# ciccio42/openvla-oft

Hardware: AMD Instinct MI355X
Metric: fine-tune samples/s (action-chunks/s) OpenVLA-7B bf16 (higher is better)
Workload: dtype bf16; 1 GPU; BASELINE.json configs[2]: LoRA r=32 fine-tune step (fwd+bwd+AdamW), 2x224x224 images + proprio, L1 head; global_batch=8, seq_len=608, parallelism=dp1, mask_mode=bidirectional

## Files before the change

### include/ovla.h

```cpp
#ifndef OVLA_H_
#define OVLA_H_

#include <stdint.h>

#ifdef __cplusplus
extern "C" {
#endif

#define OVLA_OK 0
#define OVLA_EINVAL (-1)
#define OVLA_EARCH (-2)
#define OVLA_ELAUNCH (-3)

#define OVLA_ABI_VERSION 1

const char* ovla_last_error(void);
int ovla_abi_version(void);
const char* ovla_build_hash(void);
int ovla_check_device(int device);

enum { OVLA_ACT_NONE = 0, OVLA_ACT_GELU = 1, OVLA_ACT_RELU = 2, OVLA_ACT_SILU = 3, OVLA_ACT_GELU_TANH = 4,
       OVLA_ACT_SWIGLU = 5 };

typedef struct {
  const void* A; int64_t lda;
  const void* B; int64_t ldb;
  const void* A2; int64_t lda2;
  const void* B2; int64_t ldb2;
  void* C; int64_t ldc;
  void* C_pre;
  const void* bias;
  const void* colscale;
  const void* residual; int64_t ldr;
  const void* film_gamma;
  const void* film_beta;
  int32_t film_rows;
  int32_t M, N, K, K2;
  int32_t k2_group_n;
  int32_t a_group_n;
  int32_t act;
  int32_t split_k;
  int32_t tile;
  float alpha;
  const void* dact_src; int64_t ld_dact;
  int32_t dact_mode, dact_act;
  const void* rope_cos; const void* rope_sin;
  int32_t rope_S, rope_cols;
  float* rowsq_out;
  const float* rowscale_part; int32_t rowscale_slots; float rowscale_eps; float* rowscale_r;
  uint32_t* hybrid_counters; int32_t n_hybrid_counters;
  void* workspace;
  int64_t workspace_bytes;
} ovla_gemm_args;

int ovla_gemm_plan(int32_t M, int32_t N, int32_t K, int32_t K2, int32_t k2_group_n, int64_t workspace_bytes, int32_t* tile,
                   int32_t* full_tiles, int32_t* rem_tiles, int32_t* rem_splits, double* est_seconds);
int ovla_gemm_resolved_tile(const ovla_gemm_args* a, int32_t* tile);
int64_t ovla_gemm_workspace_bytes(int32_t M, int32_t N, int32_t split_k);
int ovla_gemm_bf16(const ovla_gemm_args* a, void* stream);

typedef struct {
  int32_t tile;
  int32_t splits;
} ovla_gemm_schedule;
enum { OVLA_EPI_ROPE = 1,
       OVLA_EPI_ROWSCALE = 2,
       OVLA_EPI_SWIGLU = 4,
       OVLA_EPI_GENERAL = 8,
       OVLA_EPI_ROWSQ = 16     };
int ovla_gemm_fixed_schedule(int32_t N, int32_t K, int32_t K2, int32_t k2_group_n, int32_t epi_flags, ovla_gemm_schedule* out);
int64_t ovla_gemm_fixed_workspace_bytes(int32_t M, int32_t N, const ovla_gemm_schedule* s);
int ovla_gemm_bf16_fixed(const ovla_gemm_args* a, const ovla_gemm_schedule* s, void* stream);

typedef struct {
  const void* X; int64_t ldx;
  const void* Y; int64_t ldy;
  void* C; int64_t ldc;
  int32_t M, P, Q;
  float alpha;
  int32_t out_mode;
  float* W;
} ovla_gemm_tn_args;
int64_t ovla_gemm_tn_workspace_floats(const ovla_gemm_tn_args* a, int32_t group_size);
int ovla_gemm_tn_bf16(const ovla_gemm_tn_args* a, void* stream);
#define OVLA_TN_MAX_GROUP 4
int ovla_gemm_tn_grouped(const ovla_gemm_tn_args* problems, int32_t n, void* stream);

typedef struct {
  const void* dy; int64_t ld_dy;
  const void* Bt; int64_t ld_bt;
  const void* t;  int64_t ld_t;
  void* dt; int64_t ld_dt;
  float* dB; int64_t ld_db;
  int32_t M, gn, G, r;
  float scale;
  void* workspace; int64_t workspace_bytes;
} ovla_lora_bwd_args;
int64_t ovla_lora_bwd_workspace_bytes(int32_t M, int32_t gn, int32_t G);
int ovla_lora_bwd(const ovla_lora_bwd_args* a, void* stream);

typedef struct {
  void* t; int64_t ld;
  const int32_t* obs_slot;
  const int32_t* obs_slot_host;
  int32_t M, G, n, r, rows_per_obs, n_obs;
} ovla_lora_route_args;
int ovla_lora_route(const ovla_lora_route_args* a, void* stream);

typedef struct {
  const void* src; void* dst;
  const int32_t* obs_slot; const int32_t* obs_slot_host;
  int64_t src_slot_stride;
  int32_t n, rows, dim, rows_per_obs, n_obs, elem_bytes;
} ovla_select_by_slot_args;
int ovla_select_by_slot(const ovla_select_by_slot_args* a, void* stream);

typedef struct { const void* X; int64_t ldx; float* out; int32_t M, N; } ovla_colsum_args;
int ovla_colsum_bf16(const ovla_colsum_args* a, void* stream);

typedef struct {
  const void* Q; const void* K; const void* V; int64_t q_stride, k_stride, v_stride;
  void* O; int64_t o_stride;
  float* lse;
  const int32_t* kv_len;
  int32_t B, H, S, head_dim;
  int32_t causal;
  float scale;
} ovla_attn_fwd_args;
int ovla_attn_fwd(const ovla_attn_fwd_args* a, void* stream);

typedef struct {
  const void* Q; const void* K; const void* V; int64_t q_stride, k_stride, v_stride;
  const void* O; const void* dO; int64_t o_stride, do_stride;
  const float* lse;
  float* delta;
  void* dQ; void* dK; void* dV; int64_t dq_stride, dk_stride, dv_stride;
  const int32_t* kv_len;
  int32_t B, H, S, head_dim;
  int32_t causal;
  float scale;
  const void* rope_cos;
  const void* rope_sin;
} ovla_attn_bwd_args;
int ovla_attn_bwd(const ovla_attn_bwd_args* a, void* stream);

typedef struct {
  const void* x; void* y; const void* weight; const void* bias;
  float* mean; float* rstd;
  int32_t rows, dim; float eps; int32_t is_rms;
} ovla_norm_fwd_args;
int ovla_norm_fwd(const ovla_norm_fwd_args* a, void* stream);

typedef struct {
  const void* x; const void* dy; const void* weight;
  const float* mean; const float* rstd;
  void* dx; float* dweight; float* dbias;
  int32_t rows, dim; int32_t is_rms; int32_t dx_accum;
} ovla_norm_bwd_args;
int ovla_norm_bwd(const ovla_norm_bwd_args* a, void* stream);

int ovla_rope_table(void* cos_table, void* sin_table, int32_t S, int32_t head_dim, float theta, void* stream);
typedef struct {
  void* qk; int64_t ld; int32_t rows, S, n_heads, head_dim;
  const void* cos_table; const void* sin_table; int32_t inverse;
} ovla_rope_args;
int ovla_rope(const ovla_rope_args* a, void* stream);

typedef struct { const void* gu; void* h; int32_t rows, F; } ovla_swiglu_fwd_args;
int ovla_swiglu_fwd(const ovla_swiglu_fwd_args* a, void* stream);
typedef struct { const void* gu; const void* dh; void* dgu; int32_t rows, F; } ovla_swiglu_bwd_args;
int ovla_swiglu_bwd(const ovla_swiglu_bwd_args* a, void* stream);

typedef struct { const void* z; const void* dh; void* dz; int64_t n; int32_t act; } ovla_act_bwd_args;
int ovla_act_bwd(const ovla_act_bwd_args* a, void* stream);

typedef struct { const void* a; const void* b; void* out; int64_t n; } ovla_add_args;
int ovla_add_bf16(const ovla_add_args* a, void* stream);
typedef struct { const void* x; const void* scale; void* out; int32_t rows, dim; } ovla_colscale_args;
int ovla_colscale_bf16(const ovla_colscale_args* a, void* stream);

typedef struct { const void* pixels; void* out; int64_t ldo; int32_t B, C_total, c0, H, W, patch, n_img, img_cstride; } ovla_im2col_args;
int ovla_im2col(const ovla_im2col_args* a, void* stream);

typedef struct { const void* src; void* dst; int32_t n_img, H, W, out, crop; float crop_scale; float mean[6]; float std[6]; } ovla_image_prep_args;
int ovla_image_prep(const ovla_image_prep_args* a, void* stream);

typedef struct {
  const void* src; void* dst; void* workspace; int64_t workspace_bytes;
  const int32_t* row_starts; const float* row_weights; const int32_t* col_starts; const float* col_weights;
  int32_t n_img, H, W, out_h, out_w, row_span, col_span;
} ovla_image_resize_args;
int64_t ovla_image_resize_workspace_bytes(int32_t n_img, int32_t W, int32_t out_h);
int ovla_image_resize(const ovla_image_resize_args* a, void* stream);

typedef struct { const void* src; void* dst; void* workspace; int64_t workspace_bytes; int32_t n_img, H, W, quality; } ovla_jpeg_roundtrip_args;
int64_t ovla_jpeg_roundtrip_workspace_bytes(int32_t n_img, int32_t H, int32_t W);
int ovla_jpeg_roundtrip(const ovla_jpeg_roundtrip_args* a, void* stream);

typedef struct {
  const void* src; void* dst; const float* params; void* workspace; int64_t workspace_bytes;
  int32_t n_img, H, W, out, ops_mask; float mean[6]; float std[6];
} ovla_image_augment_args;
int64_t ovla_image_augment_workspace_bytes(int32_t n_img, int32_t out);
int ovla_image_augment(const ovla_image_augment_args* a, void* stream);

typedef struct { const void* patches; const void* pos; const void* prefix; void* tokens; int32_t B, n_patches, n_prefix, dim; } ovla_vit_embed_args;
int ovla_vit_embed(const ovla_vit_embed_args* a, void* stream);
typedef struct {
  const void* src; void* dst; int32_t B, rows, dim;
  int64_t src_batch_stride, src_row0, src_ld, dst_batch_stride, dst_row0, dst_ld, dst_col0; int32_t accumulate;
} ovla_copy_rows_args;
int ovla_copy_rows(const ovla_copy_rows_args* a, void* stream);

typedef struct { void* dy; const void* x_pre; const void* gamma; float* dgamma; float* dbeta; int32_t B, rows_per_batch, dim; } ovla_film_bwd_args;
int ovla_film_bwd(const ovla_film_bwd_args* a, void* stream);

typedef struct { const void* x; const uint8_t* row_mask; void* out; int32_t B, L, dim; } ovla_masked_mean_args;
int ovla_masked_mean(const ovla_masked_mean_args* a, void* stream);

typedef struct { const int64_t* ids; const int64_t* labels; const void* embed_table; void* out; int32_t B, L, D, vocab; int64_t action_token_begin; } ovla_language_average_args;
int ovla_language_average(const ovla_language_average_args* a, void* stream);

typedef struct { const int64_t* ids; const int64_t* labels; const int32_t* lens; const void* embed_table; void* out; int32_t B, L, D, vocab; int64_t action_token_begin; } ovla_language_average_ragged_args;
int ovla_language_average_ragged(const ovla_language_average_ragged_args* a, void* stream);

typedef struct {
  const int64_t* ids; const int64_t* labels;
  const void* embed_table;
  const void* patches;
  const void* noisy;
  void* out;
  int32_t* action_pos;
  int32_t B, L, P, D, A, vocab;
  int32_t ignore_index, action_token_begin, action_dim;
} ovla_assemble_args;
int ovla_assemble_multimodal(const ovla_assemble_args* a, void* stream);

int ovla_row_sumsq(const void* x, int64_t ld, float* out, int32_t rows, int32_t dim, void* stream);

typedef struct { const void* src; const int32_t* index; void* dst; int32_t n, dim; int64_t src_ld, dst_ld; int32_t scatter_add; } ovla_gather_rows_args;
int ovla_gather_rows(const ovla_gather_rows_args* a, void* stream);

typedef struct {
  const void* logits; int64_t ld; const int64_t* targets; float* loss_rows; int32_t* argmax; void* dlogits; int64_t ld_d;
  int32_t rows, vocab; float grad_scale;
} ovla_token_ce_args;
int ovla_token_ce(const ovla_token_ce_args* a, void* stream);

typedef struct { const void* logits; int64_t ld; int32_t* token; int32_t* bin; int32_t rows, vocab, n_tokens, n_bins; } ovla_argmax_bins_args;
int ovla_argmax_bins(const ovla_argmax_bins_args* a, void* stream);

typedef struct {
  const void* x; const void* W; const void* b; void* pred;
  const void* target; float* loss_sum;
// ... 57 lines not shown
```

### openvla-oft_amd/engine.py

```python
from __future__ import annotations

import contextlib
import math
from typing import Dict, List, Optional

import os

import torch

from . import _lib, ops
from .config import VLAConfig, VitConfig

BF16 = torch.bfloat16
F32 = torch.float32
_FUSE = os.environ.get("OVLA_FUSE_DACT", "none")
_FUSE_ROPE_FWD = os.environ.get("OVLA_FUSE_ROPE_FWD", "1") == "1"
_GROUP_TN = os.environ.get("OVLA_GROUP_TN", "1") == "1"
_FUSE_ACT, _FUSE_SWIGLU = _FUSE in ("act", "all"), _FUSE in ("swiglu", "all")
_FUSE_HEAD = {"0": False, "1": True}.get(os.environ.get("OVLA_FUSE_HEAD", "auto"), None)
_ASYNC_UPLOAD = os.environ.get("OVLA_ASYNC_UPLOAD", "1") != "0"
_FOLD_RMSNORM = os.environ.get("OVLA_FOLD_RMSNORM", "1") != "0"
_INFER_W4 = os.environ.get("OVLA_INFER_W4", "1") != "0"
_FUSE_SWIGLU_FWD = os.environ.get("OVLA_FUSE_SWIGLU_FWD", "0") == "1"
_LORA_BWD_FUSED = os.environ.get("OVLA_LORA_BWD", "0") == "1"


class Param:

    def __init__(self, name, init: torch.Tensor):
        self.name, self.shape, self.dtype = name, tuple(init.shape), init.dtype
        self._init = init
        self.data: Optional[torch.Tensor] = None
        self.grad: Optional[torch.Tensor] = None
        self.offset = 0

    @property
    def numel(self):
        return math.prod(self.shape)


class ParamStore:
    ALIGN = 64

    def __init__(self, device):
        self.device = device
        self.params: List[Param] = []
        self.flat: Dict[torch.dtype, torch.Tensor] = {}
        self.flat_grad: Dict[torch.dtype, torch.Tensor] = {}
        self.exp_avg: Dict[torch.dtype, torch.Tensor] = {}
        self.exp_avg_sq: Dict[torch.dtype, torch.Tensor] = {}
        self.step = 0
        self.finalized = False

    def add(self, name: str, init: torch.Tensor) -> Param:
        assert not self.finalized and init.dtype in (BF16, F32)
        p = Param(name, init.to(self.device))
        self.params.append(p)
        return p

    def finalize(self):
        for dtype in (BF16, F32):
            group = [p for p in reversed(self.params) if p.dtype == dtype]
            total = 0
            for p in group:
                p.offset = total
                total += (p.numel + self.ALIGN - 1) // self.ALIGN * self.ALIGN
            if total == 0:
                continue
            flat = torch.zeros(total, dtype=dtype, device=self.device)
            grad = torch.zeros(total, dtype=F32, device=self.device)
            for p in group:
                p.data = flat[p.offset: p.offset + p.numel].view(p.shape)
                p.data.copy_(p._init)
                p.grad = grad[p.offset: p.offset + p.numel].view(p.shape)
                p._init = None
            self.flat[dtype], self.flat_grad[dtype] = flat, grad
        self.finalized = True

    def init_optimizer(self):
        for dtype, flat in self.flat.items():
            self.exp_avg[dtype] = torch.zeros_like(flat)
            self.exp_avg_sq[dtype] = torch.zeros_like(flat)
        self.step = 0

    def zero_grad(self):
        for g in self.flat_grad.values():
            g.zero_()

    def adamw_step(self, lr: float, *, beta1=0.9, beta2=0.999, eps=1e-8, weight_decay=0.01, grad_scale=1.0):
        if not self.exp_avg:
            self.init_optimizer()
        self.step += 1
        for dtype, flat in self.flat.items():
            ops.adamw(flat, self.exp_avg[dtype], self.exp_avg_sq[dtype], self.flat_grad[dtype], step=self.step, lr=lr, beta1=beta1,
                      beta2=beta2, eps=eps, weight_decay=weight_decay, grad_scale=grad_scale)

    def num_trainable(self):
        return sum(p.numel for p in self.params)

    def named(self) -> Dict[str, Param]:
        return {p.name: p for p in self.params}


MAX_SLOTS = 4


def slot_a_rows(g: int, s: int, n: int, r: int) -> slice:
    return slice((g * n + s) * r, (g * n + s + 1) * r)


def fill_slot(A_slots, B_slots, s: int, lora_A, lora_B, groups: int):
    r = lora_B.shape[1]
    n = B_slots.shape[1] // r
    for g in range(groups):
        A_slots[slot_a_rows(g, s, n, r)] = lora_A[g * r:(g + 1) * r].to(A_slots.device, A_slots.dtype)
    B_slots[:, s * r:(s + 1) * r] = lora_B.to(B_slots.device, B_slots.dtype)


class SlotRoute:

    def __init__(self):
        self.obs_slot: Optional[torch.Tensor] = None
        self.n_obs = 0
        self.host_slots: Optional[List[int]] = None


class SlotProjectors:

    def __init__(self, comps, route: SlotRoute):
        self.comps, self.route = list(comps), route

    def fwd(self, x, train: bool):
        assert not train, "multi-policy serving is inference-only"
        ys = torch.stack([c.fwd(x, False)[0] for c in self.comps])
        out = torch.zeros_like(ys[0])
        B = self.route.n_obs
        ops.select_by_slot(ys, self.route.obs_slot, rows_per_obs=1, rows=B, out=out[:B], host_slots=self.route.host_slots)
        return out, None


class LoraLinear:

    def __init__(self, store: Optional[ParamStore], name: str, W: torch.Tensor, bias: Optional[torch.Tensor], lora_A: Optional[torch.Tensor],
                 lora_B: Optional[torch.Tensor], groups: int, scale: float, need_dgrad: bool = True, ref_names=None):
        self.name, self.W, self.bias, self.groups, self.scale = name, W.contiguous(), bias, groups, scale
        self.ref_names = ref_names or [name]
        self.out_f, self.in_f = W.shape
        self.group_n = self.out_f // groups
        self.WT = ops.transpose(self.W) if need_dgrad else None
        self.has_lora = lora_A is not None
        if self.has_lora:
            self.r = lora_A.shape[0] // groups
            assert lora_A.shape == (groups * self.r, self.in_f) and lora_B.shape == (self.out_f, self.r)
            self.A = store.add(name + ".lora_A", lora_A.to(BF16))
            self.B = store.add(name + ".lora_B", lora_B.to(BF16))
            self.AT = None
            self.BT = None

    def derived_pairs(self):
        if not self.has_lora:
            return []
        dev = self.W.device
        if self.AT is None:
            self.AT = torch.empty((self.in_f, self.groups * self.r), dtype=BF16, device=dev)
            self.BT = torch.empty((self.groups * self.r, self.group_n), dtype=BF16, device=dev)
        pairs = [(self.A.data, self.AT)]
        for g in range(self.groups):
            pairs.append((self.B.data[g * self.group_n:(g + 1) * self.group_n], self.BT[g * self.r:(g + 1) * self.r]))
        return pairs

    def refresh_derived(self):
        for src, dst in self.derived_pairs():
            ops.transpose(src, dst)

    def export(self, kind: str = "data") -> Dict[str, torch.Tensor]:
        out = {}
        if self.has_lora:
            A, Bm = getattr(self.A, kind), getattr(self.B, kind)
            for g, rn in enumerate(self.ref_names):
                out[rn + ".lora_A.weight"] = A[g * self.r:(g + 1) * self.r]
                out[rn + ".lora_B.weight"] = Bm[g * self.group_n:(g + 1) * self.group_n]
        return out

    def merge(self):
        if not self.has_lora or getattr(self, "merged", False):
            return
        if self.AT is None:
            self.refresh_derived()
        gn, r = self.group_n, self.r
        for g in range(self.groups):
            Wg = self.W[g * gn:(g + 1) * gn]
            ops.gemm(self.B.data[g * gn:(g + 1) * gn], self.AT[:, g * r:(g + 1) * r], out=Wg, residual=Wg, alpha=self.scale)
        if self.WT is not None:
            ops.transpose(self.W, self.WT)
        self.merged = True

    def init_slots(self, n: int, r: int, route: "SlotRoute"):
        if self.has_lora:
            raise ValueError(f"{self.name}: adapter slots need a linear without merged or trainable adapters")
        if not 1 <= n <= MAX_SLOTS:
            raise ValueError(f"{self.name}: {n} adapter slots (1 .. {MAX_SLOTS} supported)")
        if r % 8:
            raise ValueError(f"{self.name}: slot rank {r} must be a multiple of 8")
        dev = self.W.device
        self.n_slots, self.slot_r, self.route = n, r, route
        self.A_slots = torch.zeros((self.groups * n * r, self.in_f), dtype=BF16, device=dev)
        self.B_slots = torch.zeros((self.out_f, n * r), dtype=BF16, device=dev)

    def clear_slots(self):
        self.n_slots, self.A_slots, self.B_slots = 0, None, None

    def set_slot(self, s: int, lora_A: torch.Tensor, lora_B: torch.Tensor):
        n, r, G = self.n_slots, self.slot_r, self.groups
        if not 0 <= s < n:
            raise ValueError(f"{self.name}: slot {s} of {n}")
        if tuple(lora_A.shape) != (G * r, self.in_f) or tuple(lora_B.shape) != (self.out_f, r):
            raise ValueError(f"{self.name}: adapter shapes {tuple(lora_A.shape)} / {tuple(lora_B.shape)} do not fit rank {r} "
                             f"(want {(G * r, self.in_f)} / {(self.out_f, r)})")
        fill_slot(self.A_slots, self.B_slots, s, lora_A, lora_B, G)

    def slots_active(self) -> bool:
        return bool(getattr(self, "n_slots", 0)) and self.route.obs_slot is not None

    def fwd(self, x, *, act=0, residual=None, colscale=None, c_pre=None, film=None, out=None, rope=None):
        t_s = None
        if self.slots_active():
            rt, n, r, M = self.route, self.n_slots, self.slot_r, x.shape[0]
            if M % rt.n_obs:
                raise RuntimeError(f"{self.name}: {M} rows do not divide over {rt.n_obs} observations")
            t_s = ops.gemm(x, self.A_slots, alpha=self.scale)
            ops.lora_route(t_s, rt.obs_slot, G=self.groups, n=n, r=r, rows_per_obs=M // rt.n_obs, host_slots=rt.host_slots)
            y = ops.gemm(x, self.W, out=out, bias=self.bias, act=act, residual=residual, colscale=colscale, c_pre=c_pre, film=film,
                         a2=t_s, b2=self.B_slots, k2_group_n=self.group_n if self.groups > 1 else 0, rope=rope)
            return y, None
        if self.has_lora and not getattr(self, "merged", False):
            t_s = ops.gemm(x, self.A.data, alpha=self.scale)
            y = ops.gemm(x, self.W, out=out, bias=self.bias, act=act, residual=residual, colscale=colscale, c_pre=c_pre, film=film,
                         a2=t_s, b2=self.B.data, k2_group_n=self.group_n if self.groups > 1 else 0, rope=rope)
        else:
            y = ops.gemm(x, self.W, out=out, bias=self.bias, act=act, residual=residual, colscale=colscale, c_pre=c_pre, film=film, rope=rope)
        return y, (x, t_s)

    def bwd(self, dy, saved, need_dx=True, dact=None, tn_queue=None):
        if getattr(self, "n_slots", 0):
            raise RuntimeError(f"{self.name}: this linear carries adapter slots (multi-policy serving); that path is inference-only")
        x, t_s = saved
        dx = None
        if getattr(self, "merged", False):
            raise RuntimeError(f"{self.name}: LoRA adapters were merged into the base weight; this engine is inference-only")
        if self.has_lora:
            r, G, gn = self.r, self.groups, self.group_n
            if _LORA_BWD_FUSED and r == 32 and dy.shape[0] >= 512:
                dt = ops.lora_bwd(dy, self.BT, t_s, self.B.grad, gn=gn, G=G, scale=self.scale)
                probs = [(dt, x, self.A.grad)]
            else:
                dt = ops.gemm(dy, self.BT, alpha=self.scale, a_group_n=r if G > 1 else 0)
                probs = [(dy[:, g * gn:(g + 1) * gn], t_s[:, g * r:(g + 1) * r], self.B.grad[g * gn:(g + 1) * gn]) for g in range(G)]
                probs.append((dt, x, self.A.grad))
            if tn_queue is not None:
                tn_queue.extend(probs)
            else:
                ops.gemm_tn_grouped(probs)
            if need_dx:
                dx = ops.gemm(dy, self.WT, a2=dt, b2=self.AT, dact=dact)
        elif need_dx:
            dx = ops.gemm(dy, self.WT, dact=dact)
        return dx


class FullLinear:

    def __init__(self, store: ParamStore, name: str, W: torch.Tensor, bias: Optional[torch.Tensor], master_fp32: bool = False):
        dt = F32 if master_fp32 else BF16
        self.name, self.master_fp32 = name, master_fp32
        self.out_f, self.in_f = W.shape
        self.in_pad = (self.in_f + 7) // 8 * 8
        Wp = torch.zeros((self.out_f, self.in_pad), dtype=dt, device=W.device)
        Wp[:, : self.in_f] = W.to(dt)
        self.W = store.add(name + ".weight", Wp)
        self.b = store.add(name + ".bias", bias.to(dt)) if bias is not None else None
        self.Wc = self.bc = None

    def derived_pairs(self):
        return []

    def refresh_derived(self):
        if self.master_fp32:
            self.Wc = ops.cvt_f32_to_bf16(self.W.data, self.Wc)
            if self.b is not None:
                self.bc = ops.cvt_f32_to_bf16(self.b.data, self.bc)
        else:
            self.Wc, self.bc = self.W.data, (None if self.b is None else self.b.data)

    def export(self, kind: str = "data") -> Dict[str, torch.Tensor]:
        out = {self.name + ".weight": getattr(self.W, kind)[:, : self.in_f]}
        if self.b is not None:
            out[self.name + ".bias"] = getattr(self.b, kind)
        return out

    def fwd(self, x, *, act=0, residual=None, c_pre=None, split_k=1):
        y = ops.gemm(x, self.Wc, bias=self.bc, act=act, residual=residual, c_pre=c_pre, split_k=split_k)
        return y, (x,)

    def bwd(self, dy, saved, need_dx=True):
        (x,) = saved
        M = dy.shape[0]
        ops.gemm_tn(dy, x, out=self.W.grad)
        if self.b is not None:
            ops.colsum(dy, self.b.grad)
        if not need_dx:
            return None
        if M % 8 != 0:
            raise RuntimeError(f"{self.name}: row count {M} must be a multiple of 8 for the data gradient")
        dyT = ops.transpose(dy)
        return ops.gemm_tn(dyT, self.Wc, accumulate=False, out_dtype=BF16)


ACT_ID = {"gelu": ops.ACT_GELU, "gelu_tanh": ops.ACT_GELU_TANH}


def lora_predicate(lora, has):
    if lora == "auto":
        if has is None:
            raise ValueError('lora="auto" needs the state dict\'s `has`')

        def pred(names):
            flags = [has(n + ".lora_A.weight") for n in names]
            if any(flags) != all(flags):
                raise ValueError(f"LoRA adapters present for only some of the fused linears {names}")
            return flags[0]

        return pred
    return lambda names: bool(lora)


class VitTower:
    def __init__(self, store, prefix: str, vc: VitConfig, get, cfg: VLAConfig, lora, film: bool = False):
        self.vc, self.prefix = vc, prefix
        lora = lora if callable(lora) else lora_predicate(lora, None)
        w = get(prefix + "patch_embed.proj.weight").reshape(vc.dim, -1)
        self.patch_w = torch.zeros((vc.dim, vc.patch_k), dtype=BF16, device=w.device)
        self.patch_w[:, : w.shape[1]] = w
        self.patch_b = get(prefix + "patch_embed.proj.bias")
        self.pos = get(prefix + "pos_embed").reshape(vc.n_patches, vc.dim).contiguous()
        pre = []
        if vc.n_prefix > 0:
            pre.append(get(prefix + "cls_token").reshape(1, vc.dim))
            if vc.n_prefix > 1:
                pre.append(get(prefix + "reg_token").reshape(vc.n_prefix - 1, vc.dim))
        self.prefix_tokens = torch.cat(pre, 0).contiguous() if pre else None
        self.act = ACT_ID[vc.act]
        self.blocks = []
        s = cfg.lora_scale

        def L(name, groups=1):
            A = get(name + ".lora_A.weight") if lora([name]) else None
            Bm = get(name + ".lora_B.weight") if lora([name]) else None
            return LoraLinear(store, name, get(name + ".weight"), get(name + ".bias"), A, Bm, groups, s)

        self.film = film
        for i in range(vc.depth - 1):
            p = f"{prefix}blocks.{i}."
            fl = None
            if film:
                fl = (FullLinear(store, p + "scale", get(p + "scale.weight").float(), get(p + "scale.bias").float(), master_fp32=True),
                      FullLinear(store, p + "shift", get(p + "shift.weight").float(), get(p + "shift.bias").float(), master_fp32=True))
            blk = dict(film=fl, ln1_w=get(p + "norm1.weight"), ln1_b=get(p + "norm1.bias"), ln2_w=get(p + "norm2.weight"), ln2_b=get(p + "norm2.bias"),
                       qkv=L(p + "attn.qkv"), proj=L(p + "attn.proj"), fc1=L(p + "mlp.fc1"), fc2=L(p + "mlp.fc2"),
                       ls1=get(p + "ls1.scale_factor") if vc.layerscale else None, ls2=get(p + "ls2.scale_factor") if vc.layerscale else None)
            self.blocks.append(blk)

    def linears(self):
        for b in self.blocks:
            yield from (b["qkv"], b["proj"], b["fc1"], b["fc2"])
            if b["film"] is not None:
                yield from b["film"]

    def export_frozen(self) -> Dict[str, torch.Tensor]:
        vc, p = self.vc, self.prefix
        out = {p + "patch_embed.proj.weight": self.patch_w[:, : 3 * vc.patch * vc.patch].reshape(vc.dim, 3, vc.patch, vc.patch),
               p + "patch_embed.proj.bias": self.patch_b, p + "pos_embed": self.pos.reshape(1, vc.n_patches, vc.dim)}
        if self.prefix_tokens is not None:
            out[p + "cls_token"] = self.prefix_tokens[:1].reshape(1, 1, vc.dim)
            if vc.n_prefix > 1:
                out[p + "reg_token"] = self.prefix_tokens[1:].reshape(1, vc.n_prefix - 1, vc.dim)
        for i, b in enumerate(self.blocks):
            q = f"{p}blocks.{i}."
            out.update({q + "norm1.weight": b["ln1_w"], q + "norm1.bias": b["ln1_b"], q + "norm2.weight": b["ln2_w"], q + "norm2.bias": b["ln2_b"]})
            for nm, key in (("attn.qkv", "qkv"), ("attn.proj", "proj"), ("mlp.fc1", "fc1"), ("mlp.fc2", "fc2")):
                if getattr(b[key], "merged", False):
                    raise RuntimeError("the adapters were merged into the base weights: there is no training-time backbone state to export")
                out[q + nm + ".weight"], out[q + nm + ".bias"] = b[key].W, b[key].bias
            if b["ls1"] is not None:
                out[q + "ls1.scale_factor"], out[q + "ls2.scale_factor"] = b["ls1"], b["ls2"]
        return out

    def fwd(self, pixels, c0: int, n_img: int, train: bool, film_avg=None):
        vc = self.vc
        B = pixels.shape[0] * n_img
        cols = ops.im2col(pixels, c0, vc.patch, vc.patch_k, n_img=n_img, img_cstride=6)
        patches = ops.gemm(cols, self.patch_w, bias=self.patch_b)
        x = ops.vit_embed(patches, self.pos, self.prefix_tokens, B, vc.n_patches, vc.dim)
        T = vc.n_patches + vc.n_prefix
        H, hd = vc.heads, vc.head_dim
        saved = []
        for blk in self.blocks:
            h1, mean1, rstd1 = ops.norm_fwd(x, blk["ln1_w"], blk["ln1_b"], eps=vc.eps, rms=False, save_stats=train)
            qkv, s_qkv = blk["qkv"].fwd(h1)
            o, lse = ops.attn_fwd(qkv[:, : vc.dim], qkv[:, vc.dim: 2 * vc.dim], qkv[:, 2 * vc.dim:], B, T, H, hd)
# ... 1080 lines not shown
```

### openvla-oft_amd/ops.py

```python
from __future__ import annotations

import contextlib
import ctypes
import threading

import torch

from . import _lib
from ._lib import STRUCTS

ACT_NONE, ACT_GELU, ACT_RELU, ACT_SILU, ACT_GELU_TANH, ACT_SWIGLU = 0, 1, 2, 3, 4, 5
BF16 = torch.bfloat16

PROFILE = None


_WS_BYTES = 96 << 20
_ws_cache = {}
_ws_retired = []


def _workspace(device, nbytes):
    key = (device, torch.cuda.current_stream(device).cuda_stream)
    ws = _ws_cache.get(key)
# ... 149 lines not shown
    _lib.check(_lib.lib().ovla_gemm_resolved_tile(ctypes.byref(g), ctypes.byref(t)), "ovla_gemm_resolved_tile")
    tile = t.value % 100 if t.value >= 100 else t.value
    return f"gemm_nt_t18k{g.K2 // 32}" if tile == 18 else f"gemm_nt_t{tile}"


def gemm_tn(x, y, *, out=None, alpha=1.0, accumulate=True, out_dtype=torch.float32):
    _chk(x, name="x"); _chk(y, name="y")
    M, P = x.shape
    Q = y.shape[1]
    assert y.shape[0] == M and x.stride(1) == 1 and y.stride(1) == 1
    if out is None:
        out = torch.zeros((P, Q), dtype=out_dtype, device=x.device) if accumulate else torch.empty((P, Q), dtype=out_dtype, device=x.device)
    assert out.shape == (P, Q) and out.stride(1) == 1
    g = STRUCTS["ovla_gemm_tn_args"]()
    g.X, g.ldx, g.Y, g.ldy, g.C, g.ldc = x.data_ptr(), x.stride(0), y.data_ptr(), y.stride(0), out.data_ptr(), out.stride(0)
    g.M, g.P, g.Q, g.alpha = M, P, Q, alpha
    if accumulate:
        assert out.dtype == torch.float32
        g.out_mode = 0
    else:
        g.out_mode = 1 if out.dtype == torch.float32 else 2
    ws = _tn_workspace(g, 1, x.device)
    e0 = _prof_begin()
    _lib.call("ovla_gemm_tn_bf16", g, _stream())
    _prof_end(e0, "gemm_tn", 2.0 * M * P * Q)
    return out


_TN_WS_FLOATS = {}


def _tn_workspace(g, group_size, device):
    import ctypes

    key = (g.M, g.P, g.Q, g.out_mode, group_size)
    n = _TN_WS_FLOATS.get(key)
    if n is None:
        n = _lib.lib().ovla_gemm_tn_workspace_floats(ctypes.byref(g), group_size)
        if n < 0:
            raise _lib.OvlaError(f"ovla_gemm_tn_workspace_floats: invalid problem ({_lib.lib().ovla_last_error().decode()})")
        _TN_WS_FLOATS[key] = n
    if n == 0:
        return None
    ws = torch.empty(n, dtype=torch.float32, device=device)
    g.W = ws.data_ptr()
    return ws


def gemm_tn_grouped(problems):
    import ctypes

    n = len(problems)
    arr = (STRUCTS["ovla_gemm_tn_args"] * n)()
    ws = []
    flops = 0.0
    for i, (x, y, out) in enumerate(problems):
        _chk(x, name="x"); _chk(y, name="y")
        M, P = x.shape
        Q = y.shape[1]
        assert y.shape[0] == M and x.stride(1) == 1 and y.stride(1) == 1 and out.shape == (P, Q) and out.dtype == torch.float32
        g = arr[i]
        g.X, g.ldx, g.Y, g.ldy, g.C, g.ldc = x.data_ptr(), x.stride(0), y.data_ptr(), y.stride(0), out.data_ptr(), out.stride(0)
        g.M, g.P, g.Q, g.alpha, g.out_mode = M, P, Q, 1.0, 0
        ws.append(_tn_workspace(g, n, x.device))
        flops += 2.0 * M * P * Q
    e0 = _prof_begin()
    _lib.check(_lib.lib().ovla_gemm_tn_grouped(arr, n, _stream()), "ovla_gemm_tn_grouped")
    _prof_end(e0, "gemm_tn", flops)


def row_sumsq(x, out=None):
    _chk(x, name="x")
    rows, dim = x.shape
    assert x.stride(1) == 1 and dim % 64 == 0
    if out is None:
        out = torch.empty((rows, dim // 64), dtype=torch.float32, device=x.device)
    _lib.check(_lib.lib().ovla_row_sumsq(x.data_ptr(), x.stride(0), out.data_ptr(), rows, dim, _stream()), "ovla_row_sumsq")
    return out


def gemm_plan(M, N, K, K2=0, k2_group_n=0, workspace_bytes=_WS_BYTES):
    import ctypes

    t, f, r, sp, est = ctypes.c_int32(), ctypes.c_int32(), ctypes.c_int32(), ctypes.c_int32(), ctypes.c_double()
    _lib.check(_lib.lib().ovla_gemm_plan(M, N, K, K2, k2_group_n, ctypes.c_int64(workspace_bytes), ctypes.byref(t), ctypes.byref(f), ctypes.byref(r),
                                         ctypes.byref(sp), ctypes.byref(est)), "ovla_gemm_plan")
    return t.value, f.value, r.value, sp.value, est.value


EPI_ROPE, EPI_ROWSCALE, EPI_SWIGLU, EPI_GENERAL, EPI_ROWSQ = 1, 2, 4, 8, 16
BATCH_INVARIANT_DEFAULT = _os.environ.get("OVLA_BATCH_INVARIANT", "1") != "0"
_mode = threading.local()
_fixed_cache = {}


@contextlib.contextmanager
def batch_invariant(on: bool = True):
    prev = getattr(_mode, "invariant", False)
    _mode.invariant = bool(on)
    try:
        yield
    finally:
        _mode.invariant = prev


def batch_invariant_enabled() -> bool:
    return getattr(_mode, "invariant", False)


def _fixed_schedule_struct(N, K, K2=0, k2_group_n=0, epi=0):
    key = (N, K, K2, k2_group_n, epi)
    s = _fixed_cache.get(key)
    if s is None:
        s = STRUCTS["ovla_gemm_schedule"]()
        _lib.check(_lib.lib().ovla_gemm_fixed_schedule(N, K, K2, k2_group_n, epi, ctypes.byref(s)), "ovla_gemm_fixed_schedule")
        _fixed_cache[key] = s
    return s


def gemm_fixed_schedule(N, K, K2=0, k2_group_n=0, epi=0):
    s = _fixed_schedule_struct(N, K, K2, k2_group_n, epi)
    return s.tile, s.splits


def gemm_fixed_workspace_bytes(M, N, sched):
    if isinstance(sched, tuple):
        s = STRUCTS["ovla_gemm_schedule"]()
        s.tile, s.splits = sched
        sched = s
    return int(_lib.lib().ovla_gemm_fixed_workspace_bytes(M, N, ctypes.byref(sched)))


def lora_bwd(dy, Bt, t, dB_grad, *, gn, G, scale, dt=None):
    _chk(dy, name="dy"); _chk(Bt, name="Bt"); _chk(t, name="t")
    M = dy.shape[0]
    r = Bt.shape[0] // G
    assert dy.shape[1] == G * gn and Bt.shape == (G * r, gn) and t.shape == (M, G * r) and dB_grad.shape == (G * gn, r) and dB_grad.dtype == torch.float32
    assert dy.stride(1) == 1 and Bt.stride(1) == 1 and t.stride(1) == 1 and dB_grad.stride(1) == 1
    if dt is None:
        dt = torch.empty((M, G * r), dtype=BF16, device=dy.device)
    need = _lib.lib().ovla_lora_bwd_workspace_bytes(M, gn, G)
    ws = _workspace(dy.device, need)
    g = STRUCTS["ovla_lora_bwd_args"]()
    g.dy, g.ld_dy, g.Bt, g.ld_bt, g.t, g.ld_t = dy.data_ptr(), dy.stride(0), Bt.data_ptr(), Bt.stride(0), t.data_ptr(), t.stride(0)
    g.dt, g.ld_dt, g.dB, g.ld_db = dt.data_ptr(), dt.stride(0), dB_grad.data_ptr(), dB_grad.stride(0)
    g.M, g.gn, g.G, g.r, g.scale = M, gn, G, r, scale
    g.workspace, g.workspace_bytes = ws.data_ptr(), ws.numel() * 4
    e0 = _prof_begin()
    _lib.call("ovla_lora_bwd", g, _stream())
    _prof_end(e0, "lora_bwd", 4.0 * M * G * gn * r)
    return dt


def transpose_table(pairs, device):
    import ctypes

    T = STRUCTS["ovla_transpose_args"]
    arr = (T * len(pairs))()
    starts = [0]
    for i, (src, dst) in enumerate(pairs):
        rows, cols = src.shape
        assert dst.shape == (cols, rows) and src.stride(1) == 1 and dst.stride(1) == 1
        arr[i].src, arr[i].dst, arr[i].rows, arr[i].cols, arr[i].lds, arr[i].ldd = src.data_ptr(), dst.data_ptr(), rows, cols, src.stride(0), dst.stride(0)
        starts.append(starts[-1] + ((rows + 63) // 64) * ((cols + 63) // 64))
    raw = torch.frombuffer(bytearray(bytes(arr)), dtype=torch.uint8).to(device)
    tile_start = torch.tensor(starts, dtype=torch.int32).to(device)
    return dict(table=raw, tile_start=tile_start, n=len(pairs), total=starts[-1], keep=pairs)


def transpose_batched(tab):
    import ctypes

    ptr = ctypes.cast(ctypes.c_void_p(tab["table"].data_ptr()), ctypes.POINTER(STRUCTS["ovla_transpose_args"]))
    _lib.check(_lib.lib().ovla_transpose_batched(ptr, tab["tile_start"].data_ptr(), tab["n"], tab["total"], _stream()), "ovla_transpose_batched")


def colsum(x, out):
    _chk(x); _chk(out, torch.float32)
    g = STRUCTS["ovla_colsum_args"]()
    g.X, g.ldx, g.out, g.M, g.N = x.data_ptr(), x.stride(0), out.data_ptr(), x.shape[0], x.shape[1]
    _lib.call("ovla_colsum_bf16", g, _stream())
    return out


def attn_fwd(q, k, v, B, S, H, hd, *, kv_len=None, causal=False, scale=None, out=None):
    for t in (q, k, v):
        _chk(t)
        assert t.stride(1) == 1 and t.shape[0] == B * S
    if out is None:
        out = torch.empty((B * S, H * hd), dtype=BF16, device=q.device)
    lse = torch.empty((B, H, S), dtype=torch.float32, device=q.device)
    g = STRUCTS["ovla_attn_fwd_args"]()
    g.Q, g.K, g.V, g.q_stride, g.k_stride, g.v_stride = q.data_ptr(), k.data_ptr(), v.data_ptr(), q.stride(0), k.stride(0), v.stride(0)
    g.O, g.o_stride, g.lse, g.kv_len = out.data_ptr(), out.stride(0), lse.data_ptr(), _p(kv_len)
    g.B, g.H, g.S, g.head_dim, g.causal = B, H, S, hd, int(causal)
    g.scale = float(scale if scale is not None else hd ** -0.5)
    e0 = _prof_begin()
    _lib.call("ovla_attn_fwd", g, _stream())
    _prof_end(e0, "attn_fwd", 4.0 * B * H * S * S * hd * (0.5 if causal else 1.0))
    return out, lse


def attn_bwd(q, k, v, o, do, lse, B, S, H, hd, *, kv_len=None, causal=False, scale=None, dq=None, dk=None, dv=None, rope=None):
    for t in (q, k, v, o, do):
        _chk(t)
        assert t.stride(1) == 1
    dev = q.device
    if dq is None:
        dq = torch.empty((B * S, H * hd), dtype=BF16, device=dev)
    if dk is None:
        dk = torch.empty((B * S, H * hd), dtype=BF16, device=dev)
    if dv is None:
        dv = torch.empty((B * S, H * hd), dtype=BF16, device=dev)
    delta = torch.empty((B, H, S), dtype=torch.float32, device=dev)
    g = STRUCTS["ovla_attn_bwd_args"]()
    g.Q, g.K, g.V, g.q_stride, g.k_stride, g.v_stride = q.data_ptr(), k.data_ptr(), v.data_ptr(), q.stride(0), k.stride(0), v.stride(0)
    g.O, g.dO, g.o_stride, g.do_stride = o.data_ptr(), do.data_ptr(), o.stride(0), do.stride(0)
    g.lse, g.delta = lse.data_ptr(), delta.data_ptr()
    g.dQ, g.dK, g.dV, g.dq_stride, g.dk_stride, g.dv_stride = dq.data_ptr(), dk.data_ptr(), dv.data_ptr(), dq.stride(0), dk.stride(0), dv.stride(0)
    g.kv_len = _p(kv_len)
    g.B, g.H, g.S, g.head_dim, g.causal = B, H, S, hd, int(causal)
    g.scale = float(scale if scale is not None else hd ** -0.5)
    if rope is not None:
        assert rope[0].shape[0] >= S and rope[0].shape[1] == hd // 2 and rope[0].is_contiguous() and rope[1].is_contiguous()
        g.rope_cos, g.rope_sin = rope[0].data_ptr(), rope[1].data_ptr()
    e0 = _prof_begin()
    _lib.call("ovla_attn_bwd", g, _stream())
    _prof_end(e0, "attn_bwd", 10.0 * B * H * S * S * hd * (0.5 if causal else 1.0))
    return dq, dk, dv


def norm_fwd(x, weight, bias=None, *, eps, rms, out=None, save_stats=True):
    _chk(x); _chk(weight)
    rows, dim = x.shape
    assert x.is_contiguous()
    if out is None:
        out = torch.empty_like(x)
    mean = torch.empty(rows, dtype=torch.float32, device=x.device) if (save_stats and not rms) else None
    rstd = torch.empty(rows, dtype=torch.float32, device=x.device) if save_stats else None
    g = STRUCTS["ovla_norm_fwd_args"]()
    g.x, g.y, g.weight, g.bias, g.mean, g.rstd = x.data_ptr(), out.data_ptr(), weight.data_ptr(), _p(bias), _p(mean), _p(rstd)
    g.rows, g.dim, g.eps, g.is_rms = rows, dim, eps, int(rms)
    _lib.call("ovla_norm_fwd", g, _stream())
    return out, mean, rstd


def norm_bwd(x, dy, weight, mean, rstd, *, rms, dx=None, dx_accum=False, dweight=None, dbias=None):
    _chk(x); _chk(dy)
    rows, dim = x.shape
    assert x.is_contiguous() and dy.is_contiguous()
    if dx is None:
        assert not dx_accum
        dx = torch.empty_like(x)
    g = STRUCTS["ovla_norm_bwd_args"]()
    g.x, g.dy, g.weight, g.mean, g.rstd, g.dx = x.data_ptr(), dy.data_ptr(), weight.data_ptr(), _p(mean), rstd.data_ptr(), dx.data_ptr()
    g.dweight, g.dbias, g.rows, g.dim, g.is_rms, g.dx_accum = _p(dweight), _p(dbias), rows, dim, int(rms), int(dx_accum)
    _lib.call("ovla_norm_bwd", g, _stream())
    return dx


def rope_table(S, hd, theta, device):
    cos = torch.empty((S, hd // 2), dtype=BF16, device=device)
    sin = torch.empty((S, hd // 2), dtype=BF16, device=device)
    _lib.check(_lib.lib().ovla_rope_table(cos.data_ptr(), sin.data_ptr(), S, hd, theta, _stream()), "ovla_rope_table")
    return cos, sin


def rope_(qk, S, n_heads, hd, cos, sin, inverse=False):
    _chk(qk)
    g = STRUCTS["ovla_rope_args"]()
    g.qk, g.ld, g.rows, g.S, g.n_heads, g.head_dim = qk.data_ptr(), qk.stride(0), qk.shape[0], S, n_heads, hd
    g.cos_table, g.sin_table, g.inverse = cos.data_ptr(), sin.data_ptr(), int(inverse)
    _lib.call("ovla_rope", g, _stream())
    return qk


def swiglu_fwd(gu, out=None):
    _chk(gu)
    rows, F2 = gu.shape
    h = torch.empty((rows, F2 // 2), dtype=BF16, device=gu.device) if out is None else out
    assert h.shape == (rows, F2 // 2) and h.dtype == BF16 and h.is_contiguous()
    g = STRUCTS["ovla_swiglu_fwd_args"]()
    g.gu, g.h, g.rows, g.F = gu.data_ptr(), h.data_ptr(), rows, F2 // 2
    _lib.call("ovla_swiglu_fwd", g, _stream())
    return h


def swiglu_bwd(gu, dh, out=None):
    _chk(gu); _chk(dh)
    rows, F2 = gu.shape
    dgu = torch.empty_like(gu) if out is None else out
    assert dgu.shape == gu.shape and dgu.dtype == BF16 and dgu.is_contiguous()
    g = STRUCTS["ovla_swiglu_bwd_args"]()
    g.gu, g.dh, g.dgu, g.rows, g.F = gu.data_ptr(), dh.data_ptr(), dgu.data_ptr(), rows, F2 // 2
    _lib.call("ovla_swiglu_bwd", g, _stream())
    return dgu


def act_bwd(z, dh, act, out=None):
    _chk(z); _chk(dh)
    assert z.is_contiguous() and dh.is_contiguous()
    dz = torch.empty_like(z) if out is None else out
    assert dz.shape == z.shape and dz.dtype == BF16 and dz.is_contiguous()
    g = STRUCTS["ovla_act_bwd_args"]()
    g.z, g.dh, g.dz, g.n, g.act = z.data_ptr(), dh.data_ptr(), dz.data_ptr(), z.numel(), act
    _lib.call("ovla_act_bwd", g, _stream())
# ... 385 lines not shown
```

Measured before the change: 48.25 samples/s.

## Add streaming split-K skinny GEMM kernel for LoRA down-projections

Adds a dedicated HIP kernel for the skinny LoRA projections (x·Aᵀ in forward, dy·Bᵀ in backward, N ≤ 128). It uses a deep global-to-LDS ring buffer with swizzled tiles and MFMA, plus split-K with an fp32 workspace and a separate reduce kernel, so that many CUs stream the large-K operand. The generic GEMM tiles poorly on such narrow outputs. The new path is used by default for r=32 layers with large dimensions and M≥512. The cost is an extra reduce launch and workspace traffic when the problem is split.

Result: no change. 48.55 samples/s, median of 6 (+0.6%).

```diff
diff --git a/include/ovla.h b/include/ovla.h
--- a/include/ovla.h
+++ b/include/ovla.h
@@ -100,6 +100,17 @@
 int ovla_lora_bwd(const ovla_lora_bwd_args* a, void* stream);
 
 typedef struct {
+  const void* A; int64_t lda;
+  const void* B; int64_t ldb;
+  void* C; int64_t ldc;
+  int32_t M, N, K, groups;
+  float alpha;
+  void* workspace; int64_t workspace_bytes;
+} ovla_lora_proj_args;
+int32_t ovla_lora_proj_splits(int32_t M, int32_t N, int32_t K, int32_t groups, int64_t workspace_bytes);
+int ovla_lora_proj(const ovla_lora_proj_args* a, void* stream);
+
+typedef struct {
   void* t; int64_t ld;
   const int32_t* obs_slot;
   const int32_t* obs_slot_host;
diff --git a/openvla-oft_amd/csrc/lora_proj.hip b/openvla-oft_amd/csrc/lora_proj.hip
--- /dev/null
+++ b/openvla-oft_amd/csrc/lora_proj.hip
@@ -0,0 +1,199 @@
+#include "common.h"
+
+namespace {
+
+constexpr int PBK = 64;
+constexpr int PBM = 64;
+
+struct ProjParams {
+  const bf16_bits *A, *B;
+  int64_t lda, ldb, ldc;
+  bf16_bits* C;
+  float* ws;
+  int M, N, K, T, splits, chunk;
+  float alpha;
+};
+
+template <int N>
+OVLA_DEV void proj_wait_vmcnt() {
+  asm volatile("s_waitcnt vmcnt(%0)" ::"n"(N) : "memory");
+}
+
+OVLA_DEV bf16x8_bits proj_frag(const bf16_bits* tile, int row, int chunk) {
+  const int phys = chunk ^ ((row >> 1) & 7);
+  return *reinterpret_cast<const bf16x8_bits*>(tile + row * PBK + phys * 8);
+}
+
+template <int NT, int RING>
+__global__ __launch_bounds__(256) void lora_proj_kernel(const ProjParams p) {
+  constexpr int NB = NT * 16;
+  constexpr int STAGE_ELEMS = (PBM + NB) * PBK;
+  constexpr int PA = PBM / 8 / 4, PB = NB / 8 / 4;
+  constexpr int G = PA + PB;
+  constexpr int D = RING - 1;
+  static_assert(PB * 32 == NB && RING >= 2 && RING <= 5 && 3 * G < 64, "tile shape");
+  extern __shared__ __attribute__((aligned(16))) char smem_raw[];
+  bf16_bits* smem = reinterpret_cast<bf16_bits*>(smem_raw);
+
+  const int tid = threadIdx.x, lane = tid & 63;
+  const int wave = __builtin_amdgcn_readfirstlane(tid >> 6);
+  const int m0 = blockIdx.x * PBM, split = blockIdx.y, grp = blockIdx.z;
+  const int t_begin = split * p.chunk;
+  const int t_end = (t_begin + p.chunk) < p.T ? (t_begin + p.chunk) : p.T;
+  const bf16_bits* Ag = p.A + (int64_t)grp * p.K;
+  const bf16_bits* Bg = p.B + (int64_t)grp * NB * p.ldb;
+  const int n_base = grp * NB;
+
+  const bf16_bits *srcA[PA], *srcB[PB];
+#pragma unroll
+  for (int i = 0; i < PA; ++i) {
+    const int r = (wave * PA + i) * 8 + (lane >> 3);
+    const int c = (lane & 7) ^ ((r >> 1) & 7);
+    int gr = m0 + r;
+    gr = gr < p.M - 1 ? gr : p.M - 1;
+    srcA[i] = Ag + (int64_t)gr * p.lda + c * 8;
+  }
+#pragma unroll
+  for (int i = 0; i < PB; ++i) {
+    const int r = (wave * PB + i) * 8 + (lane >> 3);
+    const int c = (lane & 7) ^ ((r >> 1) & 7);
+    srcB[i] = Bg + (int64_t)r * p.ldb + c * 8;
+  }
+  auto stage = [&](int t) {
+    bf16_bits* sA = smem + ((t - t_begin) % RING) * STAGE_ELEMS;
+    bf16_bits* sB = sA + PBM * PBK;
+#pragma unroll
+    for (int i = 0; i < PA; ++i)
+      __builtin_amdgcn_global_load_lds((const __attribute__((address_space(1))) void*)(srcA[i] + (int64_t)t * PBK),
+                                       (__attribute__((address_space(3))) void*)(sA + (wave * PA + i) * 8 * PBK), 16, 0, 0);
+#pragma unroll
+    for (int i = 0; i < PB; ++i)
+      __builtin_amdgcn_global_load_lds((const __attribute__((address_space(1))) void*)(srcB[i] + (int64_t)t * PBK),
+                                       (__attribute__((address_space(3))) void*)(sB + (wave * PB + i) * 8 * PBK), 16, 0, 0);
+  };
+
+  f32x4 acc[NT];
+#pragma unroll
+  for (int j = 0; j < NT; ++j) acc[j] = f32x4{0.f, 0.f, 0.f, 0.f};
+
+#pragma unroll
+  for (int s = 0; s < D; ++s)
+    if (t_begin + s < t_end) stage(t_begin + s);
+
+  const int arow = wave * 16 + (lane & 15), brl = lane & 15, cq = lane >> 4;
+  for (int t = t_begin; t < t_end; ++t) {
+    const int newer = (t_end - 1 - t) < (D - 1) ? (t_end - 1 - t) : (D - 1);
+    if (newer >= 3) proj_wait_vmcnt<3 * G>();
+    else if (newer == 2) proj_wait_vmcnt<2 * G>();
+    else if (newer == 1) proj_wait_vmcnt<G>();
+    else proj_wait_vmcnt<0>();
+    __builtin_amdgcn_s_barrier();
+    if (t + D < t_end) stage(t + D);
+    const bf16_bits* sA = smem + ((t - t_begin) % RING) * STAGE_ELEMS;
+    const bf16_bits* sB = sA + PBM * PBK;
+#pragma unroll
+    for (int s = 0; s < 2; ++s) {
+      const bf16x8_bits a = proj_frag(sA, arow, s * 4 + cq);
+      bf16x8_bits b[NT];
+#pragma unroll
+      for (int j = 0; j < NT; ++j) b[j] = proj_frag(sB, j * 16 + brl, s * 4 + cq);
+#pragma unroll
+      for (int j = 0; j < NT; ++j) acc[j] = __builtin_amdgcn_mfma_f32_16x16x32_bf16(b[j], a, acc[j], 0, 0, 0);
+    }
+  }
+  asm volatile("s_waitcnt vmcnt(0)" ::: "memory");
+
+  const int m = m0 + arow;
+  if (m >= p.M) return;
+#pragma unroll
+  for (int j = 0; j < NT; ++j) {
+    const int n = n_base + j * 16 + 4 * cq;
+    if (p.splits > 1) {
+      *reinterpret_cast<f32x4*>(p.ws + ((int64_t)split * p.M + m) * p.N + n) = acc[j];
+    } else {
+      bf16x4_bits o;
+#pragma unroll
+      for (int e = 0; e < 4; ++e) o[e] = (short)f2bf(acc[j][e] * p.alpha);
+      *reinterpret_cast<bf16x4_bits*>(p.C + (int64_t)m * p.ldc + n) = o;
+    }
+  }
+}
+
+template <int S>
+__global__ __launch_bounds__(256) void lora_proj_reduce_kernel(const ProjParams p) {
+  const int64_t quads = (int64_t)p.M * (p.N / 4);
+  const int64_t q = (int64_t)blockIdx.x * 256 + threadIdx.x;
+  if (q >= quads) return;
+  const int m = (int)(q / (p.N / 4));
+  const int n = (int)(q % (p.N / 4)) * 4;
+  f32x4 w[S];
+#pragma unroll
+  for (int s = 0; s < S; ++s) w[s] = *reinterpret_cast<const f32x4*>(p.ws + ((int64_t)s * p.M + m) * p.N + n);
+  f32x4 v = {0.f, 0.f, 0.f, 0.f};
+#pragma unroll
+  for (int s = 0; s < S; ++s) v += w[s];
+  bf16x4_bits o;
+#pragma unroll
+  for (int e = 0; e < 4; ++e) o[e] = (short)f2bf(v[e] * p.alpha);
+  *reinterpret_cast<bf16x4_bits*>(p.C + (int64_t)m * p.ldc + n) = o;
+}
+
+int lora_proj_splits(int M, int N, int K, int groups, int64_t workspace_bytes) {
+  const int T = K / PBK;
+  const int tiles = (groups > 1 || N == 32) ? cdiv(M, 128) * (N / 32) : cdiv(M, 64);
+  int sp = 1;
+  while (sp < 8 && tiles * sp < 256 && (sp * 2) * 8 <= T && (int64_t)(sp * 2) * M * N * 4 <= workspace_bytes) sp *= 2;
+  return sp;
+}
+
+template <int NT, int RING>
+int launch_proj(const ProjParams& p, int groups, hipStream_t stream) {
+  constexpr int lds = RING * (PBM + NT * 16) * PBK * 2;
+  static const hipError_t attr = hipFuncSetAttribute((const void*)lora_proj_kernel<NT, RING>, hipFuncAttributeMaxDynamicSharedMemorySize, lds);
+  if (attr != hipSuccess) {
+    ovla_set_error("ovla_lora_proj: %d bytes of LDS refused: %s", lds, hipGetErrorString(attr));
+    return OVLA_ELAUNCH;
+  }
+  hipLaunchKernelGGL((lora_proj_kernel<NT, RING>), dim3(cdiv(p.M, PBM), p.splits, groups), dim3(256), lds, stream, p);
+  OVLA_CHECK_LAUNCH("ovla_lora_proj");
+  return OVLA_OK;
+}
+
+}
+
+extern "C" int32_t ovla_lora_proj_splits(int32_t M, int32_t N, int32_t K, int32_t groups, int64_t workspace_bytes) {
+  if (M < 1 || N < 32 || K < PBK || (K % PBK) || groups < 1) return -1;
+  return lora_proj_splits(M, N, K, groups, workspace_bytes);
+}
+
+extern "C" int ovla_lora_proj(const ovla_lora_proj_args* a, void* stream_) {
+  hipStream_t stream = (hipStream_t)stream_;
+  OVLA_REQUIRE(a && a->A && a->B && a->C, "ovla_lora_proj: null pointer");
+  OVLA_REQUIRE(a->M > 0 && a->K > 0 && (a->K % PBK) == 0, "ovla_lora_proj: M = %d, K = %d (K must be a positive multiple of %d)", a->M, a->K, PBK);
+  OVLA_REQUIRE(a->N == 32 || a->N == 64 || a->N == 96 || a->N == 128, "ovla_lora_proj: N = %d (32, 64, 96 or 128)", a->N);
+  OVLA_REQUIRE(a->groups == 1 || (a->groups > 1 && a->groups * 32 == a->N), "ovla_lora_proj: groups = %d needs N = 32 * groups (block-diagonal form, 32 columns per group)", a->groups);
+  OVLA_REQUIRE(a->lda >= (int64_t)a->groups * a->K && a->ldb >= a->K && a->ldc >= a->N, "ovla_lora_proj: leading dimension smaller than extent (lda >= groups * K, ldb >= K, ldc >= N)");
+  OVLA_REQUIRE((a->lda % 8) == 0 && (a->ldb % 8) == 0 && (a->ldc % 4) == 0 && aligned16(a->A) && aligned16(a->B) && (((uintptr_t)a->C) & 7) == 0,
+               "ovla_lora_proj: A / B need 16-byte alignment and lda, ldb multiples of 8; C 8-byte alignment and ldc a multiple of 4");
+  const int64_t wsb = a->workspace ? a->workspace_bytes : 0;
+  OVLA_REQUIRE(!a->workspace || aligned16(a->workspace), "ovla_lora_proj: the workspace needs 16-byte alignment");
+  ProjParams p;
+  p.A = (const bf16_bits*)a->A; p.B = (const bf16_bits*)a->B; p.C = (bf16_bits*)a->C;
+  p.lda = a->lda; p.ldb = a->ldb; p.ldc = a->ldc;
+  p.ws = (float*)a->workspace;
+  p.M = a->M; p.N = a->N; p.K = a->K; p.T = a->K / PBK; p.alpha = a->alpha;
+  p.splits = lora_proj_splits(a->M, a->N, a->K, a->groups, wsb);
+  p.chunk = cdiv(p.T, p.splits);
+  int rc;
+  if (a->groups > 1 || a->N == 32) rc = launch_proj<2, 4>(p, a->groups, stream);
+  else if (a->N == 64) rc = launch_proj<4, 5>(p, 1, stream);
+  else if (a->N == 96) rc = launch_proj<6, 4>(p, 1, stream);
+  else rc = launch_proj<8, 3>(p, 1, stream);
+  if (rc != OVLA_OK || p.splits <= 1) return rc;
+  const dim3 rgrid(cdiv((int64_t)p.M * (p.N / 4), 256));
+  if (p.splits == 2) hipLaunchKernelGGL(lora_proj_reduce_kernel<2>, rgrid, dim3(256), 0, stream, p);
+  else if (p.splits == 4) hipLaunchKernelGGL(lora_proj_reduce_kernel<4>, rgrid, dim3(256), 0, stream, p);
+  else hipLaunchKernelGGL(lora_proj_reduce_kernel<8>, rgrid, dim3(256), 0, stream, p);
+  OVLA_CHECK_LAUNCH("ovla_lora_proj(reduce)");
+  return OVLA_OK;
+}
diff --git a/openvla-oft_amd/engine.py b/openvla-oft_amd/engine.py
--- a/openvla-oft_amd/engine.py
+++ b/openvla-oft_amd/engine.py
@@ -23,6 +23,7 @@
 _INFER_W4 = os.environ.get("OVLA_INFER_W4", "1") != "0"
 _FUSE_SWIGLU_FWD = os.environ.get("OVLA_FUSE_SWIGLU_FWD", "0") == "1"
 _LORA_BWD_FUSED = os.environ.get("OVLA_LORA_BWD", "0") == "1"
+_LORA_STREAM = os.environ.get("OVLA_LORA_STREAM", "1") != "0"
 
 
 class Param:
@@ -156,6 +157,8 @@
             self.B = store.add(name + ".lora_B", lora_B.to(BF16))
             self.AT = None
             self.BT = None
+            self.stream_proj = (_LORA_STREAM and self.r == 32 and groups * self.r <= 128 and min(self.in_f, self.group_n) >= 4096
+                                and self.in_f % 64 == 0 and self.group_n % 64 == 0)
 
     def derived_pairs(self):
         if not self.has_lora:
@@ -234,7 +237,10 @@
                          a2=t_s, b2=self.B_slots, k2_group_n=self.group_n if self.groups > 1 else 0, rope=rope)
             return y, None
         if self.has_lora and not getattr(self, "merged", False):
-            t_s = ops.gemm(x, self.A.data, alpha=self.scale)
+            if self.stream_proj and x.shape[0] >= 512 and not ops.batch_invariant_enabled():
+                t_s = ops.lora_proj(x, self.A.data, alpha=self.scale)
+            else:
+                t_s = ops.gemm(x, self.A.data, alpha=self.scale)
             y = ops.gemm(x, self.W, out=out, bias=self.bias, act=act, residual=residual, colscale=colscale, c_pre=c_pre, film=film,
                          a2=t_s, b2=self.B.data, k2_group_n=self.group_n if self.groups > 1 else 0, rope=rope)
         else:
@@ -254,7 +260,10 @@
                 dt = ops.lora_bwd(dy, self.BT, t_s, self.B.grad, gn=gn, G=G, scale=self.scale)
                 probs = [(dt, x, self.A.grad)]
             else:
-                dt = ops.gemm(dy, self.BT, alpha=self.scale, a_group_n=r if G > 1 else 0)
+                if self.stream_proj and dy.shape[0] >= 512:
+                    dt = ops.lora_proj(dy, self.BT, alpha=self.scale, groups=G)
+                else:
+                    dt = ops.gemm(dy, self.BT, alpha=self.scale, a_group_n=r if G > 1 else 0)
                 probs = [(dy[:, g * gn:(g + 1) * gn], t_s[:, g * r:(g + 1) * r], self.B.grad[g * gn:(g + 1) * gn]) for g in range(G)]
                 probs.append((dt, x, self.A.grad))
             if tn_queue is not None:
diff --git a/openvla-oft_amd/ops.py b/openvla-oft_amd/ops.py
--- a/openvla-oft_amd/ops.py
+++ b/openvla-oft_amd/ops.py
@@ -325,6 +325,24 @@
     return dt
 
 
+def lora_proj(a, b, *, alpha=1.0, groups=1, out=None):
+    _chk(a, name="a"); _chk(b, name="b")
+    M, (N, K) = a.shape[0], b.shape
+    assert a.shape[1] == groups * K and a.stride(1) == 1 and b.stride(1) == 1, f"lora_proj: {a.shape} vs {b.shape} in {groups} group(s)"
+    if out is None:
+        out = torch.empty((M, N), dtype=BF16, device=a.device)
+    assert out.shape == (M, N) and out.stride(1) == 1 and out.dtype == BF16
+    ws = _workspace(a.device, _WS_BYTES)
+    g = STRUCTS["ovla_lora_proj_args"]()
+    g.A, g.lda, g.B, g.ldb, g.C, g.ldc = a.data_ptr(), a.stride(0), b.data_ptr(), b.stride(0), out.data_ptr(), out.stride(0)
+    g.M, g.N, g.K, g.groups, g.alpha = M, N, K, groups, alpha
+    g.workspace, g.workspace_bytes = ws.data_ptr(), ws.numel() * 4
+    e0 = _prof_begin()
+    _lib.call("ovla_lora_proj", g, _stream())
+    _prof_end(e0, "lora_proj", 2.0 * M * N * K)
+    return out
+
+
 def transpose_table(pairs, device):
     import ctypes
 
```
